# DanecLacey/basic_iterative_solvers

Hardware: AMD Instinct MI355X
Metric: CG iterations/sec + SpMV GFLOP/s (% HBM roofline), HPCG 256^3 at 1/2/4/8 GPUs (higher is better)
Workload: dtype f64

## Files before the change

basic_iterative_solvers_amd/csrc/bis_blas1.hip:

```cpp
#include "bis_internal.hpp"

#include <algorithm>
#include <cstdlib>

namespace {

constexpr int kEwThreads = 256;
constexpr int kMaxEwBlocks = 16384;

inline int ew_grid(int64_t n_items) {
    int64_t g = (n_items + kEwThreads - 1) / kEwThreads;
    if (g < 1) g = 1;
    if (g > kMaxDotBlocks) g = kMaxDotBlocks;
    return (int)g;
}
inline int ew_grid_wide(int64_t n_items) {
    int64_t g = (n_items + kEwThreads - 1) / kEwThreads;
    if (g < 1) g = 1;
    if (g > kMaxEwBlocks) g = kMaxEwBlocks;
    return (int)g;
}

typedef double ew_v2d_t __attribute__((ext_vector_type(2)));
__device__ __forceinline__ double2 ld_stream(const double2 *p) {
// ... 130 lines not shown
    int64_t i = (int64_t)blockIdx.x * kEwThreads + threadIdx.x;
    double acc0 = 0.0, acc1 = 0.0;
    if (VEC) {
        const int64_t n2 = n >> 1;
        double2 *w2 = reinterpret_cast<double2 *>(w);
        const double2 *u2 = reinterpret_cast<const double2 *>(u);
        const double2 *v2 = reinterpret_cast<const double2 *>(v);
        for (; i < n2; i += stride) {
            double2 wv = ld_stream(w2 + i);
            const double2 uv = ld_stream(u2 + i);
            wv.x = ew_apply<OP_SUB>(wv.x, uv.x, s);
            wv.y = ew_apply<OP_SUB>(wv.y, uv.y, s);
            w2[i] = wv;
            const double2 vv = v ? ld_stream(v2 + i) : wv;
            acc0 = fma(wv.x, vv.x, acc0);
            acc1 = fma(wv.y, vv.y, acc1);
        }
        if ((n & 1) && blockIdx.x == 0 && threadIdx.x == 0) {
            const double t = ew_apply<OP_SUB>(w[n - 1], u[n - 1], s);
            w[n - 1] = t;
            acc0 = fma(t, v ? v[n - 1] : t, acc0);
        }
    } else {
        for (; i < n; i += stride) {
            const double t = ew_apply<OP_SUB>(w[i], u[i], s);
            w[i] = t;
            acc0 = fma(t, v ? v[i] : t, acc0);
        }
    }
    const double r = block_sum<kEwThreads>(acc0 + acc1, lds);
    if (threadIdx.x == 0) partials[blockIdx.x] = r;
}

__global__ __launch_bounds__(256) void reduce_finish_kernel(const double *partials,
                                                            int n_partials, size_t stride,
                                                            double *result) {
    __shared__ double lds[4];
    const double *p = partials + (size_t)blockIdx.x * stride;
    double acc = 0.0;
    for (int i = threadIdx.x; i < n_partials; i += 256) acc += p[i];
    const double s = block_sum<256>(acc, lds);
    if (threadIdx.x == 0) result[blockIdx.x] = s;
}

enum { SC_DIV, SC_RATIO_PRODUCT, SC_SQRT_INV };
__global__ void scalar_kernel(int op, double *out, double *out2, const double *a, const double *b, const double *c,
                              const double *d) {
    if (op == SC_DIV) *out = *a / *b;
    else if (op == SC_RATIO_PRODUCT) *out = (*a / *b) * (*c / *d);
    else { const double nrm = sqrt(*a); *out = nrm; *out2 = 1.0 / nrm; }
}

}

bis_status bis_reduce_finish(bis_ctx *ctx, int n_partials, int n_values, size_t stride,
                             double *result_dev) {
    hipLaunchKernelGGL(reduce_finish_kernel, dim3(n_values), dim3(256), 0, ctx->stream,
                       ctx->partials, n_partials, stride, result_dev);
    BIS_HIP_CHECK(ctx, hipGetLastError());
    return BIS_OK;
}

bis_status bis_ensure_partials(bis_ctx *ctx, size_t n) {
    if (n <= ctx->partials_cap) return BIS_OK;
    BIS_HIP_CHECK(ctx, hipStreamSynchronize(ctx->stream));
    if (ctx->partials) BIS_HIP_CHECK(ctx, hipFree(ctx->partials));
    ctx->partials = nullptr;
    ctx->partials_cap = 0;
    BIS_HIP_CHECK(ctx, hipMalloc(&ctx->partials, sizeof(double) * n));
    ctx->partials_cap = n;
    return BIS_OK;
}

bis_status bis_fault_check(bis_ctx *ctx) {
    volatile unsigned *f = ctx->fault_host;
    if (!f || *f == 0) return BIS_OK;
    *f = 0;
    ctx->err = "a triangular sweep lost a hand-off: a row waited for a result that was never published "
               "(a workgroup of the persistent grid could not become resident, or the dependency data is corrupt); "
               "the vectors written since the last blocking call are invalid";
    return BIS_ERR_SYNC;
}

#define BIS_OPTIONS_ENV(X) X(spmv_variant) X(spmv_window) X(spmv_chunk) X(spmv_chunk_fused) X(spmv_xcd_remap) X(trsv_grid) X(ilu0_wgs) X(trsv_wave_wgs) X(trsv_trial) X(trsv_one_xcd) X(trsv_host_analysis) X(ilu0_wave) X(spmv_packed) X(spmv_packed32) X(spmv_valdict) X(spmv_sellwin) X(device_share) X(spmv_sellwin_rows) X(spmv_sellwin_joint) X(spmv_sellwin_pairs) X(spmv_sellwin_masks) X(spmv_colslab) X(spmv_win8) X(spmv_win8_rows) X(spmv_win8_depth) X(spmv_win8_implicit) X(spmv_win8_tune) X(grid_autodetect) X(tune_placement) X(force_rp64) X(trsv_tiled) X(trsv_chain) X(trsv_tile_rows) X(trsv_tile_wgs) X(trsv_tile_edge) X(trsv_tile_backoff)
#define BIS_OPTIONS_API(Y) Y(trsv_batch) Y(trsv_wave) Y(ilu0_persistent) Y(trsv_by_pos) Y(spmv_lds_pad) Y(trsv_chain_idle) Y(trsv_chain_pause) Y(trsv_chain_pairs) Y(trsv_chain_prefix) Y(trsv_tile_exp) Y(cg_nt_x) Y(spmv_sellwin_nt) Y(dist_host_plan) Y(trsv_inject_loss) Y(trsv_inject_oom) Y(trsm_form)

namespace {
std::string &opts_env_seen() { static std::string s; return s; }
std::string upper_env(const char *name) {
    std::string e = "BIS_";
    for (const char *c = name; *c; ++c) e += (char)((*c >= 'a' && *c <= 'z') ? *c - 32 : *c);
    return e;
}
}

bis_options &bis_opts() {
    static bis_options o = [] {
        bis_options v;
#define X(name) { const std::string en = upper_env(#name); if (const char *e = getenv(en.c_str())) { v.name = atoi(e); \
                  std::string &seen = opts_env_seen(); if (!seen.empty()) seen += ' '; seen += en + "=" + e; } }
        BIS_OPTIONS_ENV(X)
#undef X
        return v;
    }();
    return o;
}

extern "C" {

bis_status bis_set_option(const char *name, int value) {
    if (!name) return BIS_ERR_INVALID;
    bis_options &o = bis_opts();
#define X(opt) if (!strcmp(name, #opt)) { o.opt = value; return BIS_OK; }
    BIS_OPTIONS_ENV(X)
    BIS_OPTIONS_API(X)
#undef X
    return BIS_ERR_INVALID;
}

int bis_options_describe(char *buf, int cap) {
    const bis_options &o = bis_opts();
    std::string s = "{";
    bool first = true;
#define X(opt) if (o.opt != -1) { if (!first) s += ", "; first = false; s += std::string("\"") + #opt + "\": " + std::to_string(o.opt); }
    BIS_OPTIONS_ENV(X)
    BIS_OPTIONS_API(X)
#undef X
    if (!first) s += ", ";
    s += "\"env\": \"";
    for (char c : opts_env_seen()) if (c != '"' && c != '\\' && (unsigned char)c >= 32) s += c;
    s += "\"}";
    if (buf && cap > 0) { const int n = std::min((int)s.size(), cap - 1); memcpy(buf, s.data(), (size_t)n); buf[n] = 0; }
    return (int)s.size();
}

int bis_abi_version(void) { return 1; }

bis_status bis_ctx_create(int device, void *stream, bis_ctx **out) {
    if (!out) return BIS_ERR_INVALID;
    *out = nullptr;
    int count = 0;
    if (hipGetDeviceCount(&count) != hipSuccess || count <= 0) return BIS_ERR_NO_DEVICE;
    if (device < 0 || device >= count) return BIS_ERR_NO_DEVICE;
    if (hipSetDevice(device) != hipSuccess) return BIS_ERR_NO_DEVICE;
    hipDeviceProp_t prop;
    if (hipGetDeviceProperties(&prop, device) != hipSuccess) return BIS_ERR_NO_DEVICE;
    bis_ctx *ctx = new bis_ctx;
    ctx->device = device;
    ctx->n_cus = prop.multiProcessorCount;
    ctx->arch = prop.gcnArchName;
    ctx->hbm_bytes = (int64_t)prop.totalGlobalMem;
    if (ctx->arch.rfind("gfx950", 0) != 0) {
        fprintf(stderr, "bis_hip: device %d is %s, this library is built for gfx950 only\n",
                device, ctx->arch.c_str());
        delete ctx;
        return BIS_ERR_NO_DEVICE;
    }
    if (stream) {
        ctx->stream = (hipStream_t)stream;
    } else {
        if (hipStreamCreateWithFlags(&ctx->stream, hipStreamNonBlocking) != hipSuccess) {
            delete ctx;
            return BIS_ERR_HIP;
        }
        ctx->own_stream = true;
    }
    ctx->partials_cap = std::max((size_t)kMaxReduceBlocks * 4, (size_t)kMaxDotBlocks * 2);
// ... 327 lines not shown
```

basic_iterative_solvers_amd/csrc/bis_internal.hpp:

```cpp
#pragma once

#include <hip/hip_runtime.h>

#include <cstdint>
#include <cstdio>
#include <cstring>
#include <map>
#include <string>
#include <vector>

#include "bis_hip.h"

struct bis_trsv_plan;
struct bis_trsv_tiled;
struct bis_trsv_chain;
struct bis_trsm_plan;
struct bis_trsv_side {
    bis_trsv_plan *level = nullptr;
    bis_trsv_tiled *tiled = nullptr;
    bis_trsv_chain *chain = nullptr;
    bis_trsm_plan *multi = nullptr;
    bool tiled_tried = false, chain_tried = false;
    const char *kernel = "";
    const char *kernel_m = "";
// ... 3 lines not shown
    int type = 0;
    const bis_mat *A = nullptr;
    double *B = nullptr, *C = nullptr;
    int64_t size_B = 0, size_C = 0;
    const double *D = nullptr;
    bool upper = false;
};

struct bis_ctx {
    int device = 0;
    hipStream_t stream = nullptr;
    bool own_stream = false;
    int n_cus = 0;
    std::string arch;
    int64_t hbm_bytes = 0;
    std::string err;

    double *partials = nullptr;
    size_t partials_cap = 0;
    double *scalars_dev = nullptr;
    double *scalars_host = nullptr;
    unsigned *counters = nullptr;
    unsigned *fault_host = nullptr, *fault_dev = nullptr;

    std::map<std::string, bis_named_kernel> kernels;

    const int *spmv_stop = nullptr;

    bool profile = false;
    std::vector<std::pair<hipEvent_t, hipEvent_t>> prof_events;
    size_t prof_used = 0;
    std::vector<std::pair<hipEvent_t, hipEvent_t>> prof_sweep_events;
    size_t prof_sweep_used = 0;
};

struct bis_options;
bis_options &bis_opts();
struct bis_options {
    int spmv_variant = -1;
    int spmv_window = -1;
    int spmv_chunk = -1;
    int spmv_chunk_fused = -1;
    int spmv_xcd_remap = -1;
    int trsv_grid = -1;
    int ilu0_wave = -1;
    int ilu0_wgs = -1;
    int ilu0_persistent = -1;
    int trsv_host_analysis = -1;
    int trsv_wave = -1;
    int trsv_wave_wgs = -1;
    int trsv_trial = -1;
    int trsv_batch = -1;
    int trsv_by_pos = -1;
    int trsv_one_xcd = -1;
    int tune_placement = -1;
    int spmv_packed32 = -1;
    int spmv_lds_pad = -1;
    int spmv_packed = -1;
    int spmv_valdict = -1;
    int dist_host_plan = -1;
    int grid_autodetect = -1;
    int trsv_chain = -1;
    int trsv_chain_idle = -1;
    int trsv_chain_pause = -1;
    int trsv_chain_prefix = -1;
    int trsv_chain_pairs = -1;
    int trsv_tiled = -1;
    int trsv_tile_rows = -1;
    int trsv_tile_wgs = -1;
    int trsv_tile_backoff = -1;
    int spmv_sellwin_nt = -1;
    int cg_nt_x = -1;
    int trsv_tile_exp = -1;
    int trsv_tile_edge = -1;
    int force_rp64 = -1;
    int spmv_sellwin = -1;
    int spmv_sellwin_rows = -1;
    int spmv_sellwin_pairs = -1;
    int spmv_sellwin_joint = -1;
    int spmv_colslab = -1;
    int spmv_win8 = -1;
    int spmv_win8_rows = -1;
    int spmv_win8_depth = -1;
    int spmv_win8_implicit = -1;
    int spmv_win8_tune = -1;
    int spmv_sellwin_masks = -1;
    int device_share = -1;
    int trsm_form = -1;
    int trsv_inject_oom = -1;
    int trsv_inject_loss = -1;
};
inline bool bis_want_rp64(int64_t nnz) { return nnz >= (int64_t)INT32_MAX - 8 || bis_opts().force_rp64 > 0; }

constexpr int kMaxReduceBlocks = 2048;
constexpr int kMaxDotBlocks = 8192;
constexpr int kWinMaxTiles = 128;
constexpr int kWinTile = 16;
constexpr int kWinTileLog = 4;
constexpr int kSwRows = 256;
constexpr int kSwMaxR = 4;

struct bis_mat {
    int64_t n_rows = 0, n_cols = 0, nnz = 0;
    bool rp64 = false;
    bool view = false;
    void *row_ptr = nullptr;
    int32_t *col = nullptr;
    double *val = nullptr;
    int32_t *blk_row = nullptr;
    int64_t *blk_nnz = nullptr;
    uint16_t *loc = nullptr;
    int32_t *tiles = nullptr;
    int32_t *tile_cnt = nullptr;
    int64_t loc_base = 0;
    int max_tiles = 0;
    bool win_ok = false;
    int n_blocks = 0;
    uint16_t *pk[2] = {nullptr, nullptr};
    int32_t *pk_seg[2] = {nullptr, nullptr};
    int64_t pk_base[2] = {0, 0};
    int pk_state[2] = {0, 0};
    int pk_kind[2] = {0, 0};
    uint8_t *vcode = nullptr;
    double *vdict = nullptr;
    int64_t vd_base = 0;
    int vd_state = 0, vd_n = 0;
    double *vdiag = nullptr;
    bool vd_diag = false;
    bool vd_rm_only = false;
    int64_t view_row0 = 0;
    int64_t *rm_nnz = nullptr;
    uint16_t *rm_pk = nullptr;
    int32_t *rm_seg = nullptr;
    int64_t rm_base = 0;
    int rm_state = 0, rm_blocks = 0, rm_kind = 1;
    struct bis_sellwin *sw = nullptr;
    int sw_state = 0;
    struct bis_sellwin *sw8 = nullptr;
    std::vector<bis_mat *> *colslabs = nullptr;
    int cs_state = 0;
    double cs_trial_ms[2] = {0.0, 0.0};
    int sw8_state = 0;
    int32_t *blkf_row = nullptr;
    int64_t *blkf_nnz = nullptr;
    int n_blocks_f = 0;
    int chunk_f = 0;
    int chunk_nnz = 0;
    int max_row_nnz = 0;
    int64_t max_block_nnz = 0;
    int64_t grid[4] = {0, 0, 0, 0};
    bis_trsv_side trsv[2];
    const char *spmv_kernel[2] = {"", ""};
    const char *ilu0_kernel = "";
    const char *itrsv_kernel = "";
    const char *spmm_kernel = "";
};

#define BIS_HIP_CHECK(ctx, call)                                               \
    do {                                                                       \
        hipError_t e_ = (call);                                                \
        if (e_ != hipSuccess) {                                                \
            (ctx)->err = std::string(#call) + ": " + hipGetErrorString(e_);    \
            return BIS_ERR_HIP;                                                \
        }                                                                      \
    } while (0)

// ... 166 lines not shown
```

basic_iterative_solvers_amd/csrc/bis_spmv_sell.hip:

```cpp
#include <algorithm>
#include <cstring>
#include <cstdio>
#include <cstdlib>
#include <vector>

#include <rocprim/rocprim.hpp>

#include "bis_internal.hpp"

struct bis_sellwin {
    int n_blocks = 0;
    int64_t n_slices = 0, total_chunks = 0;
    int32_t *hdr = nullptr;
    int64_t *slice_chunk0 = nullptr;
    int32_t *own_rank = nullptr;
    uint32_t *codes = nullptr;
    double *dict = nullptr;
    int max_gran = 0;
    int fmt = 0;
    int uniform_chunks = 0;
    int n_pairs = 0, pair_stride = 0, diag_pair = -1;
    int16_t *blk_base = nullptr;
    unsigned long long *pair_key = nullptr;
    uint16_t *row_of = nullptr;
// ... 1270 lines not shown
        if (PHASE == 2) implicit = slice_rec[slice + 1] == slice_rec[slice];
        for (int c = 0; c < nch && (PHASE != 1 || implicit); ++c) {
            unsigned cc[4];
            double vv[4];
#pragma unroll
            for (int q = 0; q < 4; ++q) {
                const int j = 4 * c + q;
                cc[q] = 0;
                vv[q] = 1.0;
                if (j < len) {
                    const int ci = col[rs + j];
                    const int g = ci >> 3;
                    int lo = 0, hi = nr - 1;
                    while (lo < hi) {
                        const int mid = (lo + hi + 1) >> 1;
                        if (g0s[mid] <= g) lo = mid; else hi = mid - 1;
                    }
                    cc[q] = (unsigned)(2 + (rk[lo] + (g - g0s[lo])) * 8 + (ci & 7)) * 8u;
                    if (PHASE != 1) vv[q] = val[rs + j];
                }
            }
            unsigned base[4];
#pragma unroll
            for (int q = 0; q < 4; ++q) base[q] = 4 * c + q < len ? (cc[q] - 8u * (unsigned)in_block) & 0xffffu : 1u;
            if (PHASE == 1) {
#pragma unroll
                for (int q = 0; q < 4; ++q)
                    if (__ballot(base[q] != (unsigned)__builtin_amdgcn_readfirstlane((int)base[q])) != 0ull) implicit = false;
            } else if (PHASE == 0) {
                unsigned char *p = stream + (size_t)(c0 + c) * kW8ChunkBytes;
                *reinterpret_cast<uint2 *>(p + lane * 8) = make_uint2(cc[0] | cc[1] << 16, cc[2] | cc[3] << 16);
                *reinterpret_cast<double2 *>(p + 512 + lane * 16) = make_double2(vv[0], vv[1]);
                *reinterpret_cast<double2 *>(p + 1536 + lane * 16) = make_double2(vv[2], vv[3]);
            } else {
                unsigned char *p = stream + (size_t)(c0 + c) * kW8ValBytes;
                *reinterpret_cast<double2 *>(p + lane * 16) = make_double2(vv[0], vv[1]);
                *reinterpret_cast<double2 *>(p + 1024 + lane * 16) = make_double2(vv[2], vv[3]);
                if (!implicit) *reinterpret_cast<uint2 *>(side + (size_t)(slice_rec[slice] + c) * 512 + lane * 8) = make_uint2(cc[0] | cc[1] << 16, cc[2] | cc[3] << 16);
                else if (lane == 0) desc[c0 + c] = make_uint2(base[0] | base[1] << 16, base[2] | base[3] << 16);
            }
        }
        if (PHASE == 1 && lane == 0) slice_rec[slice] = implicit ? 0 : nch;
    }
}

typedef double w8_v2d __attribute__((ext_vector_type(2)));
typedef unsigned w8_v2u __attribute__((ext_vector_type(2)));
struct W8Chunk { w8_v2u code; w8_v2d v0, v1; };

__device__ __forceinline__ W8Chunk w8_load(const unsigned char *__restrict__ stream, int64_t c, int lane) {
    const unsigned char *p = stream + (size_t)c * kW8ChunkBytes;
    W8Chunk ch;
    ch.code = __builtin_nontemporal_load(reinterpret_cast<const w8_v2u *>(p + lane * 8));
    ch.v0 = __builtin_nontemporal_load(reinterpret_cast<const w8_v2d *>(p + 512 + lane * 16));
    ch.v1 = __builtin_nontemporal_load(reinterpret_cast<const w8_v2d *>(p + 1536 + lane * 16));
    return ch;
}

__device__ __forceinline__ void w8_load_values(const unsigned char *__restrict__ stream, int64_t c, int lane, W8Chunk &ch) {
    const unsigned char *p = stream + (size_t)c * kW8ValBytes;
    ch.v0 = __builtin_nontemporal_load(reinterpret_cast<const w8_v2d *>(p + lane * 16));
    ch.v1 = __builtin_nontemporal_load(reinterpret_cast<const w8_v2d *>(p + 1024 + lane * 16));
}

typedef unsigned short w8_v2h __attribute__((ext_vector_type(2)));
__device__ __forceinline__ unsigned w8_imply(unsigned code, unsigned off2) {
    const unsigned pad = (code & 0x10001u) * 0xffffu;
    return __builtin_bit_cast(unsigned, __builtin_bit_cast(w8_v2h, code) + __builtin_bit_cast(w8_v2h, off2)) & ~pad;
}

__device__ __forceinline__ void w8_consume(const unsigned char *win, const W8Chunk &ch, double &acc) {
#pragma clang fp contract(off)
    const double x0 = *reinterpret_cast<const double *>(win + (ch.code.x & 0xffffu));
    const double x1 = *reinterpret_cast<const double *>(win + (ch.code.x >> 16));
    const double x2 = *reinterpret_cast<const double *>(win + (ch.code.y & 0xffffu));
    const double x3 = *reinterpret_cast<const double *>(win + (ch.code.y >> 16));
    const double p0 = ch.v0.x * x0, p1 = ch.v0.y * x1, p2 = ch.v1.x * x2, p3 = ch.v1.y * x3;
    acc = acc + p0;
    acc = acc + p1;
    acc = acc + p2;
    acc = acc + p3;
}

template <int MODE, int R, int D, bool IMPL>
__global__ __launch_bounds__(256) void spmv_win8_kernel(
    const double *x, double *__restrict__ y, int64_t n_rows, int64_t n_cols, int n_blocks, int remap_arg, const double *w,
    double *__restrict__ partials, const int *stop, const int32_t *__restrict__ hdr, const int64_t *__restrict__ slice_chunk0,
    const unsigned char *__restrict__ stream, int x_al16, const int32_t *__restrict__ own_rank, const uint16_t *__restrict__ row_of,
    const w8_v2u *__restrict__ desc, const unsigned char *__restrict__ side, const int64_t *__restrict__ slice_rec) {
    if (stop && stop[1]) return;
    extern __shared__ __attribute__((aligned(16))) unsigned char lds[];
    const int b = remap_arg > 0 ? xcd_remap(blockIdx.x, remap_arg)
                                : (remap_arg < -1 ? xcd_group_remap(blockIdx.x, -remap_arg) : (int)blockIdx.x);
    if (b >= n_blocks) return;
    const int tid = threadIdx.x, lane = tid & 63;
    const int wv = __builtin_amdgcn_readfirstlane(tid >> 6);
    const int hw_g = hdr[(size_t)b * 2 * kW8Runs + lane], hw_r = hdr[(size_t)b * 2 * kW8Runs + kW8Runs + lane];
    const int64_t slice0 = ((int64_t)b * 4 + wv) * R;
    const int64_t block_row0 = (int64_t)b * kSwRows * R;
    int64_t rows_of[R];
#pragma unroll
    for (int r = 0; r < R; ++r) rows_of[r] = block_row0 + row_of[(slice0 + r) * 64 + lane];
    const int64_t my_bnd = slice_chunk0[slice0 + min(lane, R)];
    auto bnd = [&](int r) {
        const unsigned lo = (unsigned)__builtin_amdgcn_readlane((int)(unsigned)(unsigned long long)my_bnd, r);
        const unsigned hi = (unsigned)__builtin_amdgcn_readlane((int)(unsigned)((unsigned long long)my_bnd >> 32), r);
        return (int64_t)(((unsigned long long)hi << 32) | lo);
    };
    const int64_t C0 = bnd(0), C1 = bnd(R);
    const int64_t c_last = max(C1 - 1, C0);
    int64_t e[R];
#pragma unroll
    for (int rr = 0; rr < R; ++rr) e[rr] = bnd(rr + 1);
    int64_t rec[R + 1];
    unsigned off2[R];
    if (IMPL) {
        const int64_t my_rec = slice_rec[slice0 + min(lane, R)];
#pragma unroll
        for (int r = 0; r <= R; ++r) {
            const unsigned lo = (unsigned)__builtin_amdgcn_readlane((int)(unsigned)(unsigned long long)my_rec, r);
            const unsigned hi = (unsigned)__builtin_amdgcn_readlane((int)(unsigned)((unsigned long long)my_rec >> 32), r);
            rec[r] = (int64_t)(((unsigned long long)hi << 32) | lo);
        }
#pragma unroll
        for (int r = 0; r < R; ++r) off2[r] = rec[r + 1] == rec[r] ? (unsigned)(rows_of[r] - block_row0) * 0x80008u : 0u;
    }
    auto load = [&](int64_t cc) {
        if (!IMPL) return w8_load(stream, cc, lane);
        W8Chunk ch;
        w8_load_values(stream, cc, lane, ch);
        int64_t rs = 0, re = 0, cs = 0;
#pragma unroll
        for (int rr = 0; rr < R; ++rr)
            if (cc >= (rr ? e[rr - 1] : C0) && cc < e[rr]) { rs = rec[rr]; re = rec[rr + 1]; cs = rr ? e[rr - 1] : C0; }
        if (re > rs) ch.code = __builtin_nontemporal_load(reinterpret_cast<const w8_v2u *>(side + (size_t)(rs + cc - cs) * 512 + lane * 8));
        else ch.code = desc[cc];
        return ch;
    };
    W8Chunk ring[D];
#pragma unroll
    for (int d = 0; d < D; ++d) ring[d] = load(min(C0 + d, c_last));
    double wr[R];
    int own = -1;
    if (MODE == 1 && own_rank) own = own_rank[b];
#pragma unroll
    for (int r = 0; r < R; ++r) {
        const int64_t row = rows_of[r];
        wr[r] = (MODE == 1 && own < 0 && row < n_rows) ? w[row] : 0.0;
    }
    if (tid == 0) *reinterpret_cast<double *>(lds) = -0.0;
    {
        const int n_runs = __popcll(__ballot((hw_r >> 16) != 0));
        unsigned char *win = lds + 16;
        for (int k = 0; k < n_runs; ++k) {
            const int g0 = __builtin_amdgcn_readlane(hw_g, k);
            const int w2 = __builtin_amdgcn_readlane(hw_r, k);
            const int rank = w2 & 0xffff, n_pieces = (w2 >> 16) * 4;
            const int j = (wv + k) & 3;
            const int p = j * 64 + lane;
            const int64_t c = (int64_t)g0 * 8 + 2 * p;
            unsigned char *dst = win + (size_t)rank * 64 + (size_t)j * 1024;
            if (p < n_pieces) {
                if (x_al16 && c + 1 < n_cols) {
                    __builtin_amdgcn_global_load_lds((const __attribute__((address_space(1))) void *)(x + c),
                                                     (__attribute__((address_space(3))) void *)dst, 16, 0, 0);
                } else {
                    double2 v;
                    v.x = c < n_cols ? x[c] : 0.0;
                    v.y = c + 1 < n_cols ? x[c + 1] : 0.0;
                    *reinterpret_cast<double2 *>(dst + lane * 16) = v;
                }
            }
        }
    }
    __syncthreads();
    if (MODE == 1 && own >= 0) {
#pragma unroll
        for (int r = 0; r < R; ++r) wr[r] = *reinterpret_cast<const double *>(lds + 16 + ((size_t)own * 8 + (wv * R + r) * 64 + lane) * 8);
    }
    double dot_acc = 0.0;
    int64_t c = C0;
    int next = 0;
    double acc = 0.0;
    unsigned cur_off = IMPL ? off2[0] : 0u;
#define W8_END_SLICES()                                                                    \
    _Pragma("unroll") for (int rr = 0; rr < R; ++rr)                                       \
        if (rr == next && c == e[rr]) {                                                    \
            const int64_t row = rows_of[rr];                                               \
            if (row < n_rows) y[row] = acc;                                                \
            if (MODE == 1) dot_acc += row < n_rows ? acc * wr[rr] : 0.0;                   \
            acc = 0.0;                                                                     \
            ++next;                                                                        \
            if (IMPL) cur_off = off2[rr + 1 < R ? rr + 1 : R - 1];                         \
        }
    W8_END_SLICES()
    while (c < C1) {
#pragma unroll
        for (int d = 0; d < D; ++d) {
            if (c < C1) {
                W8Chunk cur = ring[d];
                ring[d] = load(min(c + D, c_last));
                if (IMPL) {
                    cur.code.x = w8_imply(cur.code.x, cur_off);
                    cur.code.y = w8_imply(cur.code.y, cur_off);
                }
                w8_consume(lds, cur, acc);
                ++c;
                W8_END_SLICES()
            }
        }
    }
#undef W8_END_SLICES
    if (MODE == 1) {
        const double t = wave_sum(dot_acc);
        if (lane == 0) partials[(size_t)b * 4 + wv] = t;
    }
}

}

void bis_spmv_win8_drop(bis_mat *A) {
    if (A->sw8) {
        if (A->sw8->own_codes) A->sw8->codes = reinterpret_cast<uint32_t *>(A->sw8->own_codes);
        hipFree(A->sw8->hdr); hipFree(A->sw8->slice_chunk0); hipFree(A->sw8->own_rank); hipFree(A->sw8->codes); hipFree(A->sw8->row_of);
        hipFree(A->sw8->slice_rec);
        delete A->sw8;
        A->sw8 = nullptr;
    }
    A->sw8_state = 0;
}

int bis_spmv_win8_blocks(const bis_mat *A) { return A->sw8_state == 1 ? A->sw8->n_blocks : 0; }
int bis_spmv_win8_rows(const bis_mat *A) { return A->sw8_state == 1 ? A->sw8->R : 0; }
bool bis_spmv_win8_implied(const bis_mat *A) { return A->sw8_state == 1 && A->sw8->slice_rec != nullptr; }
int64_t bis_spmv_win8_bytes(const bis_mat *A) {
    if (A->sw8_state != 1) return 0;
    const bis_sellwin *sw = A->sw8;
    const int64_t meta = (int64_t)sw->n_blocks * (8 * kW8Runs + 2 * kSwRows * sw->R) + 8 * (sw->n_slices + 1);
    if (!bis_spmv_win8_implied(A)) return sw->total_chunks * (int64_t)kW8ChunkBytes + meta;
    return sw->total_chunks * (int64_t)kW8ValBytes + 8 * (sw->total_chunks - sw->expl_chunks) + 512 * sw->expl_chunks + meta + 8 * (sw->n_slices + 1);
}

size_t bis_spmv_win8_stream_bytes(const bis_mat *A) {
    if (A->sw8_state != 1) return 0;
    return bis_spmv_win8_implied(A) ? A->sw8->w8_end : (size_t)kW8ChunkBytes * (size_t)(A->sw8->total_chunks + 1);
}

double bis_spmv_win8_moved_bytes(const bis_mat *A) {
    if (A->sw8_state != 1) return 0.0;
    return (double)bis_spmv_win8_bytes(A) + 64.0 * (double)A->sw8->win_gran_sum + 8.0 * (double)A->n_rows;
}
bool bis_spmv_win8_fast(const bis_mat *A, double ms) {
    return A->sw8_state == 1 && ms > 0.0 && bis_spmv_win8_moved_bytes(A) / (ms * 1e-3) >= 6.6e12;
}
void *bis_spmv_win8_swap_stream(bis_mat *A, void *stream) {
    void *old = A->sw8->codes;
    A->sw8->codes = reinterpret_cast<uint32_t *>(stream);
    return old;
}

#define W8_CHECK(call)                                                         \
    do {                                                                       \
        hipError_t e_ = (call);                                                \
// ... 25 lines not shown
        (void)hipGetLastError();
    };
    const size_t nx = (size_t)std::max(A->n_cols, A->view_row0 + A->n_rows) + 2;
    if (hipMalloc(&x, sizeof(double) * nx) != hipSuccess || hipMalloc(&y, sizeof(double) * (size_t)A->n_rows) != hipSuccess ||
        hipMalloc(&part, sizeof(double) * 4 * (size_t)sw->n_blocks) != hipSuccess ||
        hipMemsetAsync(x, 0, sizeof(double) * nx, ctx->stream) != hipSuccess ||
        hipEventCreate(&e0) != hipSuccess || hipEventCreate(&e1) != hipSuccess) { cleanup(); return BIS_OK; }
    const int nb = sw->n_blocks, remap_arg = bis_spmv_remap_arg(nb), grid = bis_spmv_grid(nb);
    const bool implied = bis_spmv_win8_implied(A);
    const int mode = implied ? 1 : 0;
    const double *w = implied ? x + A->view_row0 : nullptr;
    double *partials = implied ? part : nullptr;
    auto measure = [&](double &ms) -> bool {
        for (int i = 0; i < 2; ++i) if (bis_spmv_win8_launch(ctx, A, x, y, mode, w, partials, nullptr, remap_arg, grid) != BIS_OK) return false;
        hipEventRecord(e0, ctx->stream);
        for (int i = 0; i < 5; ++i) if (bis_spmv_win8_launch(ctx, A, x, y, mode, w, partials, nullptr, remap_arg, grid) != BIS_OK) return false;
        hipEventRecord(e1, ctx->stream);
        if (hipEventSynchronize(e1) != hipSuccess) return false;
        float f = 0.f;
        hipEventElapsedTime(&f, e0, e1);
        ms = f / 5.0;
        return true;
    };
    double best = 0.0;
    if (!measure(best)) { cleanup(); ctx->err = "win8 placement tuning: launch failed"; return BIS_ERR_HIP; }
    sw->tune_first_ms = best;
    double slowest = best;
    auto fast_enough = [&](double ms) { return bis_spmv_win8_fast(A, ms) || (!implied && ms <= 0.92 * slowest); };
    int trials = 0;
    for (; trials < k && !fast_enough(best); ++trials) {
        size_t free_b = 0, total_b = 0;
        if (hipMemGetInfo(&free_b, &total_b) != hipSuccess || free_b < bytes + ((size_t)8 << 30)) break;
        void *cand = nullptr;
        if (hipMalloc(&cand, bytes) != hipSuccess) { (void)hipGetLastError(); break; }
        void *cur = bis_spmv_win8_swap_stream(A, cand);
        hipMemcpyAsync(cand, cur, bytes, hipMemcpyDeviceToDevice, ctx->stream);
        double ms = 0.0;
        if (!measure(ms)) { bis_spmv_win8_swap_stream(A, cur); losers.push_back(cand); cleanup(); ctx->err = "win8 placement tuning: launch failed"; return BIS_ERR_HIP; }
        slowest = std::max(slowest, ms);
        if (ms < best) { best = ms; losers.push_back(cur); }
        else { bis_spmv_win8_swap_stream(A, cur); losers.push_back(cand); }
    }
    sw->tune_trials = trials;
    sw->tune_kept_ms = best;
    if (getenv("BIS_WIN8_STATS")) fprintf(stderr, "win8 placement: %d re-allocation(s) of %zu bytes tried, kernel %.4f ms on the first allocation, %.4f ms on the one kept (%.0f bytes moved: %.2f TB/s)\n", trials, bytes, sw->tune_first_ms, best, bis_spmv_win8_moved_bytes(A), bis_spmv_win8_moved_bytes(A) / (best * 1e9));
    cleanup();
    return BIS_OK;
}

extern "C" BIS_API bis_status bis_mat_win8_debug_stream(bis_mat *A, void **ptr, size_t *bytes, void *set) {
    if (!A || A->sw8_state != 1) return BIS_ERR_INVALID;
    bis_sellwin *sw = A->sw8;
    if (ptr) *ptr = sw->own_codes ? sw->own_codes : (void *)sw->codes;
    if (bytes) *bytes = bis_spmv_win8_stream_bytes(A);
    if (set) { if (!sw->own_codes) sw->own_codes = (void *)sw->codes; sw->codes = reinterpret_cast<uint32_t *>(set); }
    else if (sw->own_codes) { sw->codes = reinterpret_cast<uint32_t *>(sw->own_codes); sw->own_codes = nullptr; }
    return BIS_OK;
}

extern "C" BIS_API void bis_mat_win8_layout(const bis_mat *A, int64_t *chunks, int64_t *explicit_chunks, int64_t *slices, int *blocks, int *implied) {
    const bool ok = A && A->sw8_state == 1;
    if (chunks) *chunks = ok ? A->sw8->total_chunks : 0;
    if (explicit_chunks) *explicit_chunks = ok ? A->sw8->expl_chunks : 0;
    if (slices) *slices = ok ? A->sw8->n_slices : 0;
    if (blocks) *blocks = ok ? A->sw8->n_blocks : 0;
    if (implied) *implied = ok && bis_spmv_win8_implied(A);
}

extern "C" BIS_API void bis_mat_win8_tuning(const bis_mat *A, int *trials, double *first_ms, double *kept_ms) {
    const bool ok = A && A->sw8_state == 1;
    if (trials) *trials = ok ? A->sw8->tune_trials : 0;
    if (first_ms) *first_ms = ok ? A->sw8->tune_first_ms : 0.0;
    if (kept_ms) *kept_ms = ok ? A->sw8->tune_kept_ms : 0.0;
}

static bis_status w8_try_rows(bis_ctx *ctx, bis_mat *A, int R, bool *window_too_large);

bis_status bis_spmv_win8_try(bis_ctx *ctx, bis_mat *A) {
    if (A->sw8_state != 0) return BIS_OK;
    A->sw8_state = -1;
    if (A->n_rows == 0 || A->nnz == 0 || A->n_cols >= ((int64_t)1 << 31) - 16) return BIS_OK;
    int R = bis_opts().spmv_win8_rows > 0 ? std::min(bis_opts().spmv_win8_rows, 4) : 4;
    if (R == 3) R = 2;
    while (R > 1 && A->n_rows < (int64_t)kSwRows * R * 1024) R >>= 1;
    for (;; R >>= 1) {
        bool too_large = false;
        if (bis_status st = w8_try_rows(ctx, A, R, &too_large)) return st;
        if (A->sw8_state == 1 || !too_large || R == 1 || bis_opts().spmv_win8_rows > 0) return BIS_OK;
        A->sw8_state = -1;
    }
}

static bis_status w8_try_rows(bis_ctx *ctx, bis_mat *A, int R, bool *window_too_large) {
    *window_too_large = false;
    const int64_t nb64 = (A->n_rows + (int64_t)kSwRows * R - 1) / ((int64_t)kSwRows * R);
    if (nb64 > (int64_t)1 << 26) return BIS_OK;
    const int nb = (int)nb64;
    bis_sellwin *sw = new bis_sellwin;
    A->sw8 = sw;
    sw->n_blocks = nb;
    sw->R = R;
    sw->n_slices = (int64_t)nb * 4 * R;
    sw->fmt = 5;
    int32_t *slice_chunks = nullptr;
    void *tmp = nullptr;
    int *status = (int *)ctx->counters + 52;
    W8_CHECK(hipMalloc(&sw->hdr, sizeof(int32_t) * 2 * kW8Runs * (size_t)nb));
    W8_CHECK(hipMalloc(&sw->own_rank, sizeof(int32_t) * (size_t)nb));
    W8_CHECK(hipMemsetAsync(sw->own_rank, 0xFF, sizeof(int32_t) * (size_t)nb, ctx->stream));
    W8_CHECK(hipMalloc(&sw->row_of, sizeof(uint16_t) * (size_t)nb * kSwRows * (size_t)R));
    W8_CHECK(hipMalloc(&slice_chunks, sizeof(int32_t) * (size_t)(sw->n_slices + 1)));
    W8_CHECK(hipMalloc(&sw->slice_chunk0, sizeof(int64_t) * (size_t)(sw->n_slices + 1)));
    W8_CHECK(hipMemsetAsync(status, 0, 3 * sizeof(int), ctx->stream));
    W8_CHECK(hipMemsetAsync(status + 5, 0, sizeof(int), ctx->stream));
    W8_CHECK(hipMemsetAsync(slice_chunks, 0, sizeof(int32_t) * (size_t)(sw->n_slices + 1), ctx->stream));
    W8_CHECK(hipMemsetAsync(sw->hdr, 0, sizeof(int32_t) * 2 * kW8Runs * (size_t)nb, ctx->stream));
    if (A->rp64) hipLaunchKernelGGL(w8_plan_kernel<int64_t>, dim3(nb), dim3(256), 0, ctx->stream, (const int64_t *)A->row_ptr, A->col, A->n_rows, R, kSwMaxGran, A->view_row0, sw->hdr, slice_chunks, sw->own_rank, sw->row_of, status);
    else hipLaunchKernelGGL(w8_plan_kernel<int32_t>, dim3(nb), dim3(256), 0, ctx->stream, (const int32_t *)A->row_ptr, A->col, A->n_rows, R, kSwMaxGran, A->view_row0, sw->hdr, slice_chunks, sw->own_rank, sw->row_of, status);
    W8_CHECK(hipGetLastError());
    int h[3] = {0, 0, 0};
    W8_CHECK(hipMemcpyAsync(h, status, sizeof h, hipMemcpyDeviceToHost, ctx->stream));
    const int64_t ns1 = sw->n_slices + 1;
    hipLaunchKernelGGL(sw_widen_kernel, dim3((unsigned)((ns1 + 255) / 256)), dim3(256), 0, ctx->stream, slice_chunks, sw->slice_chunk0, ns1);
    W8_CHECK(hipGetLastError());
    size_t tmp_bytes = 0;
    W8_CHECK(rocprim::exclusive_scan(nullptr, tmp_bytes, sw->slice_chunk0, sw->slice_chunk0, (int64_t)0, (size_t)ns1, rocprim::plus<int64_t>(), ctx->stream));
    W8_CHECK(hipMalloc(&tmp, tmp_bytes));
    W8_CHECK(rocprim::exclusive_scan(tmp, tmp_bytes, sw->slice_chunk0, sw->slice_chunk0, (int64_t)0, (size_t)ns1, rocprim::plus<int64_t>(), ctx->stream));
    int64_t total = 0;
    W8_CHECK(hipMemcpyAsync(&total, sw->slice_chunk0 + sw->n_slices, sizeof total, hipMemcpyDeviceToHost, ctx->stream));
    W8_CHECK(hipStreamSynchronize(ctx->stream));
    hipFree(tmp); tmp = nullptr;
    hipFree(slice_chunks); slice_chunks = nullptr;
    sw->total_chunks = total;
    sw->max_gran = h[1];
    sw->win_gran_sum = (int64_t)(unsigned)h[2];
    if (h[0] || (double)total * 256.0 > 1.12 * (double)A->nnz + 256.0 * 4 * 64) {
        if (getenv("BIS_WIN8_STATS")) fprintf(stderr, "win8 plan (R = %d): %s, %.1f %% padding: not used\n", R, h[0] ? "window not representable" : "representable", 100.0 * ((double)total * 256.0 / (double)A->nnz - 1.0));
        *window_too_large = h[0] != 0;
        bis_spmv_win8_drop(A);
        A->sw8_state = -1;
        return BIS_OK;
    }
#define W8_FILL(PHASE, STREAM, DESC, SIDE)                                                                                                        \
    do {                                                                                                                                          \
        if (A->rp64) hipLaunchKernelGGL((w8_fill_kernel<int64_t, PHASE>), dim3(nb), dim3(256), 0, ctx->stream, (const int64_t *)A->row_ptr, A->col, \
                                        A->val, A->n_rows, R, sw->hdr, sw->slice_chunk0, sw->row_of, STREAM, sw->slice_rec, DESC, SIDE);           \
        else hipLaunchKernelGGL((w8_fill_kernel<int32_t, PHASE>), dim3(nb), dim3(256), 0, ctx->stream, (const int32_t *)A->row_ptr, A->col,     \
                                A->val, A->n_rows, R, sw->hdr, sw->slice_chunk0, sw->row_of, STREAM, sw->slice_rec, DESC, SIDE);                   \
        W8_CHECK(hipGetLastError());                                                                                                              \
    } while (0)
    sw->expl_chunks = total;
    if (bis_opts().spmv_win8_implicit != 0 && total > 0) {
        W8_CHECK(hipMalloc(&sw->slice_rec, sizeof(int64_t) * (size_t)ns1));
        W8_CHECK(hipMemsetAsync(sw->slice_rec, 0, sizeof(int64_t) * (size_t)ns1, ctx->stream));
        W8_FILL(1, nullptr, nullptr, nullptr);
        tmp_bytes = 0;
        W8_CHECK(rocprim::exclusive_scan(nullptr, tmp_bytes, sw->slice_rec, sw->slice_rec, (int64_t)0, (size_t)ns1, rocprim::plus<int64_t>(), ctx->stream));
        W8_CHECK(hipMalloc(&tmp, tmp_bytes));
        W8_CHECK(rocprim::exclusive_scan(tmp, tmp_bytes, sw->slice_rec, sw->slice_rec, (int64_t)0, (size_t)ns1, rocprim::plus<int64_t>(), ctx->stream));
        int64_t expl = 0;
        W8_CHECK(hipMemcpyAsync(&expl, sw->slice_rec + sw->n_slices, sizeof expl, hipMemcpyDeviceToHost, ctx->stream));
        W8_CHECK(hipStreamSynchronize(ctx->stream));
        hipFree(tmp); tmp = nullptr;
        if (2 * (total - expl) >= total) sw->expl_chunks = expl;
        else { hipFree(sw->slice_rec); sw->slice_rec = nullptr; }
    }
    unsigned char *stream = nullptr;
    const size_t chunk_bytes = sw->slice_rec ? kW8ValBytes : kW8ChunkBytes;
    size_t stream_bytes = chunk_bytes * (size_t)(total + 1);
    if (sw->slice_rec) {
        sw->w8_desc = stream_bytes;
        sw->w8_side = sw->w8_desc + ((8 * (size_t)(total + 1) + 255) & ~(size_t)255);
        sw->w8_end = stream_bytes = sw->w8_side + 512 * (size_t)sw->expl_chunks;
    }
    W8_CHECK(hipMalloc(&stream, stream_bytes));
    sw->codes = reinterpret_cast<uint32_t *>(stream);
    W8_CHECK(hipMemsetAsync(stream + (size_t)total * chunk_bytes, 0, chunk_bytes, ctx->stream));
    if (sw->slice_rec) {
        W8_CHECK(hipMemsetAsync(stream + sw->w8_desc, 0, sw->w8_side - sw->w8_desc, ctx->stream));
        W8_FILL(2, stream, reinterpret_cast<uint2 *>(stream + sw->w8_desc), stream + sw->w8_side);
    } else {
        W8_FILL(0, stream, nullptr, nullptr);
    }
#undef W8_FILL
    A->sw8_state = 1;
    if (bis_status tst = w8_tune_placement(ctx, A)) return tst;
    if (getenv("BIS_WIN8_STATS")) fprintf(stderr, "win8 plan (R = %d): %d blocks, window <= %d granules (%zu bytes), %.1f %% padding: used; implied slots: %s, %.1f %% of %lld chunks implicit; stream at %p (%zu bytes), hdr %p\n", R, nb, sw->max_gran, (size_t)(2 + 8 * sw->max_gran) * 8, 100.0 * ((double)total * 256.0 / (double)A->nnz - 1.0), sw->slice_rec ? "built" : "not built", 100.0 * (double)(total - sw->expl_chunks) / (double)std::max<int64_t>(total, 1), (long long)total, (void *)sw->codes, bis_spmv_win8_stream_bytes(A), (void *)sw->hdr);
    return BIS_OK;
}
#undef W8_CHECK

bis_status bis_spmv_win8_launch(bis_ctx *ctx, const bis_mat *A, const double *x, double *y, int mode, const double *w,
                                double *partials, const int *stop, int remap_arg, int grid) {
    const bis_sellwin *sw = A->sw8;
    const int x_al16 = ((uintptr_t)x & 15) == 0;
    const size_t lds = (size_t)(2 + 8 * sw->max_gran) * 8;
    const unsigned char *stream = reinterpret_cast<const unsigned char *>(sw->codes);
    const int32_t *own = (mode == 1 && w == x + A->view_row0 && x_al16) ? sw->own_rank : nullptr;
    const bool ragged = (double)sw->total_chunks * 256.0 > 1.08 * (double)A->nnz;
    const int depth = bis_opts().spmv_win8_depth > 0 ? bis_opts().spmv_win8_depth : (sw->R == 4 ? (ragged ? 2 : 1) : 3);
#define W8_L3(MODE, RR, DD) do { if (sw->slice_rec) W8_L4(MODE, RR, DD, true); else W8_L4(MODE, RR, DD, false); } while (0)
#define W8_L4(MODE, RR, DD, IMPL) hipLaunchKernelGGL((spmv_win8_kernel<MODE, RR, DD, IMPL>), dim3(grid), dim3(256), lds, ctx->stream, x, y, A->n_rows, A->n_cols, \
                                               sw->n_blocks, remap_arg, w, partials, stop, sw->hdr, sw->slice_chunk0, stream, x_al16, own, sw->row_of, \
                                               reinterpret_cast<const w8_v2u *>(stream + sw->w8_desc), stream + sw->w8_side, sw->slice_rec)
#define W8_L2(MODE, RR) do { if (depth <= 1) W8_L3(MODE, RR, 1); else if (depth == 2) W8_L3(MODE, RR, 2); else if (depth == 3) W8_L3(MODE, RR, 3); else if (depth <= 5) W8_L3(MODE, RR, 4); else W8_L3(MODE, RR, 6); } while (0)
#define W8_L1(MODE) do { if (sw->R == 4) W8_L2(MODE, 4); else if (sw->R == 2) W8_L2(MODE, 2); else W8_L2(MODE, 1); } while (0)
    if (mode == 1) W8_L1(1); else W8_L1(0);
#undef W8_L1
#undef W8_L2
#undef W8_L3
#undef W8_L4
    BIS_HIP_CHECK(ctx, hipGetLastError());
    return BIS_OK;
}
```

Measured before the change: 1085.

## Add lockstep multi-row streaming path to win8 SpMV kernel

Measured after the change: 1135, median of 6. 4.6% higher.

```diff
diff --git a/basic_iterative_solvers_amd/csrc/bis_blas1.hip b/basic_iterative_solvers_amd/csrc/bis_blas1.hip
--- a/basic_iterative_solvers_amd/csrc/bis_blas1.hip
+++ b/basic_iterative_solvers_amd/csrc/bis_blas1.hip
@@ -236,7 +236,7 @@
     return BIS_ERR_SYNC;
 }
 
-#define BIS_OPTIONS_ENV(X) X(spmv_variant) X(spmv_window) X(spmv_chunk) X(spmv_chunk_fused) X(spmv_xcd_remap) X(trsv_grid) X(ilu0_wgs) X(trsv_wave_wgs) X(trsv_trial) X(trsv_one_xcd) X(trsv_host_analysis) X(ilu0_wave) X(spmv_packed) X(spmv_packed32) X(spmv_valdict) X(spmv_sellwin) X(device_share) X(spmv_sellwin_rows) X(spmv_sellwin_joint) X(spmv_sellwin_pairs) X(spmv_sellwin_masks) X(spmv_colslab) X(spmv_win8) X(spmv_win8_rows) X(spmv_win8_depth) X(spmv_win8_implicit) X(spmv_win8_tune) X(grid_autodetect) X(tune_placement) X(force_rp64) X(trsv_tiled) X(trsv_chain) X(trsv_tile_rows) X(trsv_tile_wgs) X(trsv_tile_edge) X(trsv_tile_backoff)
+#define BIS_OPTIONS_ENV(X) X(spmv_variant) X(spmv_window) X(spmv_chunk) X(spmv_chunk_fused) X(spmv_xcd_remap) X(trsv_grid) X(ilu0_wgs) X(trsv_wave_wgs) X(trsv_trial) X(trsv_one_xcd) X(trsv_host_analysis) X(ilu0_wave) X(spmv_packed) X(spmv_packed32) X(spmv_valdict) X(spmv_sellwin) X(device_share) X(spmv_sellwin_rows) X(spmv_sellwin_joint) X(spmv_sellwin_pairs) X(spmv_sellwin_masks) X(spmv_colslab) X(spmv_win8) X(spmv_win8_rows) X(spmv_win8_depth) X(spmv_win8_lockstep) X(spmv_win8_implicit) X(spmv_win8_tune) X(grid_autodetect) X(tune_placement) X(force_rp64) X(trsv_tiled) X(trsv_chain) X(trsv_tile_rows) X(trsv_tile_wgs) X(trsv_tile_edge) X(trsv_tile_backoff)
 #define BIS_OPTIONS_API(Y) Y(trsv_batch) Y(trsv_wave) Y(ilu0_persistent) Y(trsv_by_pos) Y(spmv_lds_pad) Y(trsv_chain_idle) Y(trsv_chain_pause) Y(trsv_chain_pairs) Y(trsv_chain_prefix) Y(trsv_tile_exp) Y(cg_nt_x) Y(spmv_sellwin_nt) Y(dist_host_plan) Y(trsv_inject_loss) Y(trsv_inject_oom) Y(trsm_form)
 
 namespace {
diff --git a/basic_iterative_solvers_amd/csrc/bis_internal.hpp b/basic_iterative_solvers_amd/csrc/bis_internal.hpp
--- a/basic_iterative_solvers_amd/csrc/bis_internal.hpp
+++ b/basic_iterative_solvers_amd/csrc/bis_internal.hpp
@@ -109,6 +109,7 @@
     int spmv_win8 = -1;
     int spmv_win8_rows = -1;
     int spmv_win8_depth = -1;
+    int spmv_win8_lockstep = -1;
     int spmv_win8_implicit = -1;
     int spmv_win8_tune = -1;
     int spmv_sellwin_masks = -1;
diff --git a/basic_iterative_solvers_amd/csrc/bis_spmv_sell.hip b/basic_iterative_solvers_amd/csrc/bis_spmv_sell.hip
--- a/basic_iterative_solvers_amd/csrc/bis_spmv_sell.hip
+++ b/basic_iterative_solvers_amd/csrc/bis_spmv_sell.hip
@@ -1376,8 +1376,8 @@
     acc = acc + p3;
 }
 
-template <int MODE, int R, int D, bool IMPL>
-__global__ __launch_bounds__(256) void spmv_win8_kernel(
+template <int MODE, int R, int D, bool IMPL, bool LS = false>
+__global__ __launch_bounds__(256) __attribute__((amdgpu_waves_per_eu(4))) void spmv_win8_kernel(
     const double *x, double *__restrict__ y, int64_t n_rows, int64_t n_cols, int n_blocks, int remap_arg, const double *w,
     double *__restrict__ partials, const int *stop, const int32_t *__restrict__ hdr, const int64_t *__restrict__ slice_chunk0,
     const unsigned char *__restrict__ stream, int x_al16, const int32_t *__restrict__ own_rank, const uint16_t *__restrict__ row_of,
@@ -1431,16 +1431,48 @@
         else ch.code = desc[cc];
         return ch;
     };
-    W8Chunk ring[D];
-#pragma unroll
-    for (int d = 0; d < D; ++d) ring[d] = load(min(C0 + d, c_last));
+    W8Chunk ring[LS ? 1 : D];
+    constexpr int kChunk = IMPL ? kW8ValBytes : kW8ChunkBytes, kV0 = IMPL ? 0 : 512, kV1 = IMPL ? 1024 : 1536;
+    uint64_t ls_val[R], ls_code[R];
+    unsigned ls_coff[R];
+    int ls_cstep[R], ls_len[R];
+    W8Chunk ls_a[LS ? R : 1], ls_b[LS ? R : 1];
+    const unsigned lane16 = (unsigned)lane * 16u;
+    auto request = [&](int j, W8Chunk &ch) {
+        uint64_t vo = ls_val[j], co = ls_code[j];
+        asm("" : "+s"(vo));
+        asm("" : "+s"(co));
+        ch.v0 = __builtin_nontemporal_load(reinterpret_cast<const w8_v2d *>(stream + vo + kV0 + (size_t)lane16));
+        ch.v1 = __builtin_nontemporal_load(reinterpret_cast<const w8_v2d *>(stream + vo + kV1 + (size_t)lane16));
+        if (IMPL) ch.code = *reinterpret_cast<const w8_v2u *>(stream + co + (size_t)ls_coff[j]);
+        else ch.code = __builtin_nontemporal_load(reinterpret_cast<const w8_v2u *>(stream + co + (size_t)ls_coff[j]));
+        ls_val[j] = vo + kChunk;
+        ls_code[j] = co + (uint64_t)ls_cstep[j];
+    };
+    if (LS) {
+        const uint64_t desc_off = (uint64_t)(reinterpret_cast<uintptr_t>(desc) - reinterpret_cast<uintptr_t>(stream));
+        const uint64_t side_off = (uint64_t)(reinterpret_cast<uintptr_t>(side) - reinterpret_cast<uintptr_t>(stream));
+#pragma unroll
+        for (int j = 0; j < R; ++j) {
+            const int64_t s0 = j ? e[j - 1] : C0;
+            ls_len[j] = (int)(e[j] - s0);
+            ls_val[j] = (uint64_t)s0 * kChunk;
+            if (!IMPL) { ls_code[j] = ls_val[j]; ls_coff[j] = (unsigned)lane * 8u; ls_cstep[j] = kChunk; }
+            else if (rec[j + 1] > rec[j]) { ls_code[j] = side_off + (uint64_t)rec[j] * 512; ls_coff[j] = (unsigned)lane * 8u; ls_cstep[j] = 512; }
+            else { ls_code[j] = desc_off + (uint64_t)s0 * 8; ls_coff[j] = 0u; ls_cstep[j] = 8; }
+            if (ls_len[j] > 0) request(j, ls_a[j]);
+        }
+    } else {
+#pragma unroll
+        for (int d = 0; d < D; ++d) ring[d] = load(min(C0 + d, c_last));
+    }
     double wr[R];
     int own = -1;
     if (MODE == 1 && own_rank) own = own_rank[b];
 #pragma unroll
     for (int r = 0; r < R; ++r) {
         const int64_t row = rows_of[r];
-        wr[r] = (MODE == 1 && own < 0 && row < n_rows) ? w[row] : 0.0;
+        wr[r] = (MODE == 1 && !LS && own < 0 && row < n_rows) ? w[row] : 0.0;
     }
     if (tid == 0) *reinterpret_cast<double *>(lds) = -0.0;
     {
@@ -1468,11 +1500,56 @@
         }
     }
     __syncthreads();
-    if (MODE == 1 && own >= 0) {
+    if (MODE == 1 && !LS && own >= 0) {
 #pragma unroll
         for (int r = 0; r < R; ++r) wr[r] = *reinterpret_cast<const double *>(lds + 16 + ((size_t)own * 8 + (wv * R + r) * 64 + lane) * 8);
     }
     double dot_acc = 0.0;
+    if (LS) {
+        double ls_acc[R];
+        int t_min = ls_len[0], t_max = ls_len[0];
+#pragma unroll
+        for (int j = 0; j < R; ++j) { ls_acc[j] = 0.0; t_min = min(t_min, ls_len[j]); t_max = max(t_max, ls_len[j]); }
+        auto eat = [&](int j, W8Chunk &ch) {
+            if (IMPL) {
+                ch.code.x = w8_imply(ch.code.x, off2[j]);
+                ch.code.y = w8_imply(ch.code.y, off2[j]);
+            }
+            w8_consume(lds, ch, ls_acc[j]);
+        };
+#define W8_STEP(CUR, NXT, ALL)                                                                         \
+        {                                                                                              \
+            _Pragma("unroll") for (int j = 0; j < R; ++j) if (ALL || t + 1 < ls_len[j]) request(j, NXT[j]); \
+            _Pragma("unroll") for (int j = 0; j < R; ++j) if (ALL || t < ls_len[j]) eat(j, CUR[j]);    \
+            ++t;                                                                                       \
+        }
+        int t = 0;
+        while (t + 2 < t_min) {
+            W8_STEP(ls_a, ls_b, true)
+            W8_STEP(ls_b, ls_a, true)
+        }
+        while (t < t_max) {
+            W8_STEP(ls_a, ls_b, false)
+            if (t >= t_max) break;
+            W8_STEP(ls_b, ls_a, false)
+        }
+#undef W8_STEP
+#pragma unroll
+        for (int j = 0; j < R; ++j) {
+            const int64_t row = block_row0 + row_of[(slice0 + j) * 64 + lane];
+            if (row < n_rows) y[row] = ls_acc[j];
+            if (MODE == 1) {
+                if (own >= 0) wr[j] = *reinterpret_cast<const double *>(lds + 16 + ((size_t)own * 8 + (wv * R + j) * 64 + lane) * 8);
+                else wr[j] = row < n_rows ? w[row] : 0.0;
+                dot_acc += row < n_rows ? ls_acc[j] * wr[j] : 0.0;
+            }
+        }
+        if (MODE == 1) {
+            const double ts = wave_sum(dot_acc);
+            if (lane == 0) partials[(size_t)b * 4 + wv] = ts;
+        }
+        return;
+    }
     int64_t c = C0;
     int next = 0;
     double acc = 0.0;
@@ -1664,7 +1741,7 @@
     if (A->n_rows == 0 || A->nnz == 0 || A->n_cols >= ((int64_t)1 << 31) - 16) return BIS_OK;
     int R = bis_opts().spmv_win8_rows > 0 ? std::min(bis_opts().spmv_win8_rows, 4) : 4;
     if (R == 3) R = 2;
-    while (R > 1 && A->n_rows < (int64_t)kSwRows * R * 1024) R >>= 1;
+    if (bis_opts().spmv_win8_rows <= 0) while (R > 1 && A->n_rows < (int64_t)kSwRows * R * 1024) R >>= 1;
     for (;; R >>= 1) {
         bool too_large = false;
         if (bis_status st = w8_try_rows(ctx, A, R, &too_large)) return st;
@@ -1782,14 +1859,21 @@
     const int32_t *own = (mode == 1 && w == x + A->view_row0 && x_al16) ? sw->own_rank : nullptr;
     const bool ragged = (double)sw->total_chunks * 256.0 > 1.08 * (double)A->nnz;
     const int depth = bis_opts().spmv_win8_depth > 0 ? bis_opts().spmv_win8_depth : (sw->R == 4 ? (ragged ? 2 : 1) : 3);
+    const bool lockstep = sw->R == 4 && (bis_opts().spmv_win8_lockstep >= 0 ? bis_opts().spmv_win8_lockstep > 0 : !ragged);
 #define W8_L3(MODE, RR, DD) do { if (sw->slice_rec) W8_L4(MODE, RR, DD, true); else W8_L4(MODE, RR, DD, false); } while (0)
 #define W8_L4(MODE, RR, DD, IMPL) hipLaunchKernelGGL((spmv_win8_kernel<MODE, RR, DD, IMPL>), dim3(grid), dim3(256), lds, ctx->stream, x, y, A->n_rows, A->n_cols, \
                                                sw->n_blocks, remap_arg, w, partials, stop, sw->hdr, sw->slice_chunk0, stream, x_al16, own, sw->row_of, \
                                                reinterpret_cast<const w8_v2u *>(stream + sw->w8_desc), stream + sw->w8_side, sw->slice_rec)
 #define W8_L2(MODE, RR) do { if (depth <= 1) W8_L3(MODE, RR, 1); else if (depth == 2) W8_L3(MODE, RR, 2); else if (depth == 3) W8_L3(MODE, RR, 3); else if (depth <= 5) W8_L3(MODE, RR, 4); else W8_L3(MODE, RR, 6); } while (0)
-#define W8_L1(MODE) do { if (sw->R == 4) W8_L2(MODE, 4); else if (sw->R == 2) W8_L2(MODE, 2); else W8_L2(MODE, 1); } while (0)
+#define W8_LS(MODE) do { if (sw->slice_rec) W8_L5(MODE, true); else W8_L5(MODE, false); } while (0)
+#define W8_L5(MODE, IMPL) hipLaunchKernelGGL((spmv_win8_kernel<MODE, 4, 1, IMPL, true>), dim3(grid), dim3(256), lds, ctx->stream, x, y, A->n_rows, A->n_cols, \
+                                               sw->n_blocks, remap_arg, w, partials, stop, sw->hdr, sw->slice_chunk0, stream, x_al16, own, sw->row_of, \
+                                               reinterpret_cast<const w8_v2u *>(stream + sw->w8_desc), stream + sw->w8_side, sw->slice_rec)
+#define W8_L1(MODE) do { if (lockstep) W8_LS(MODE); else if (sw->R == 4) W8_L2(MODE, 4); else if (sw->R == 2) W8_L2(MODE, 2); else W8_L2(MODE, 1); } while (0)
     if (mode == 1) W8_L1(1); else W8_L1(0);
 #undef W8_L1
+#undef W8_LS
+#undef W8_L5
 #undef W8_L2
 #undef W8_L3
 #undef W8_L4
```
